# moabarar/nemar

Measured on AMD Instinct MI355X. Metric: train images/sec (256x256 A/B pairs), higher is better.
Workload: dtype f32

## Files before the change

### include/nemar_hip.h

```cpp
#ifndef NEMAR_HIP_H
#define NEMAR_HIP_H
#include <stddef.h>

#ifdef __cplusplus
extern "C" {
#endif

#define NEMAR_OK 0
#define NEMAR_EINVAL (-1)
#define NEMAR_ELAUNCH (-2)
#define NEMAR_EWORKSPACE (-3)

int nemar_version(void);
const char* nemar_last_error(void);

#define NEMAR_GRID_EXPLICIT 0
#define NEMAR_GRID_UNET 1
#define NEMAR_GRID_AFFINE 2
int nemar_grid_sample_fwd(const float* in, const float* grid_src, int grid_mode, float* out,
                          int N, int C, int H, int W, int Ho, int Wo, void* stream);
size_t nemar_grid_sample_bwd_workspace(int N, int C, int H, int W);
size_t nemar_grid_sample_bwd_zeroed_bytes(int N, int C, int H, int W);
int nemar_grid_sample_bwd(const float* in, const float* grid_src, int grid_mode, const float* gout,
                          float* gin, int accum_gin, float* ggrid, int accum_ggrid,
// ... 77 lines not shown
int nemar_conv2d_bwd_data_ex(const float* gy, const float* w, const float* bias, int act, float slope, float* gx0, int C0,
                             float* gx1, int C1, int N, int H, int W, int K, int OH, int OW, int R, int S, int stride, int pad,
                             int pad_mode, void* workspace, size_t ws_bytes, int prepacked, void* stream,
                             const nemar_conv_extras* extras);
int nemar_conv2d_bwd_weight_ex(const float* x0, int C0, const float* x1, int C1, const float* gy, float* gw, float* gb, int N,
                               int H, int W, int K, int OH, int OW, int R, int S, int stride, int pad, int pad_mode,
                               void* workspace, size_t ws_bytes, void* stream, const nemar_conv_extras* extras);
int nemar_pack_plan_record(int plan);
int nemar_pack_plan_jobs(int plan);
size_t nemar_pack_plan_bytes(int plan);
int nemar_pack_plan_dirty(int plan);
int nemar_pack_plan_commit(int plan, void* device_buffer, size_t bytes, void* stream);
int nemar_pack_plan_run(int plan, void* stream);
int nemar_pack_plan_reset(int plan);
int nemar_last_route(void);
int nemar_config_epoch(void);
int nemar_set_max_words_lazy(int on);
int nemar_max_words_finalize(void* max_words, int samples, void* stream);
size_t nemar_conv2d_scratch(int N, int H, int W, int K, int C, int R, int S, int stride, int pad);
int nemar_absmax(const float* t, long long n, void* out_word, void* stream);
int nemar_absmax_samples(const float* t, int samples, long long per_sample, void* out_words, void* stream);
int nemar_kernel_timer(int enable);
int nemar_kernel_timer_read(double* total_ms, double* total_flop, int* launches);
size_t nemar_bias_grad_workspace(int N, int C, int HW);
int nemar_bias_grad(const float* g, float* gb, int N, int C, int HW, void* workspace, size_t ws_bytes, void* stream);

int nemar_instnorm_fwd(const float* x, const float* residual, float* y, float* stats, int planes, int HW,
                       float eps, int act, float slope, void* stream);
int nemar_instnorm_bwd(const float* x, const float* stats, const float* gy, float* gx, int planes, int HW,
                       int act, float slope, void* stream);
// ... 108 lines not shown
```

### nemar_amd/_lib.py

```python
import ctypes as C
import os

import torch

_HERE = os.path.dirname(os.path.abspath(__file__))
PRODUCT_PATH = os.path.join(_HERE, "lib", "libnemar_hip.so")
AB_PATH = os.path.join(_HERE, "lib", "libnemar_hip_ab.so")
DEFAULT_PATH = AB_PATH if (os.environ.get("NEMAR_AB_LIBRARY") == "1" or os.environ.get("NEMAR_TUNE")) else PRODUCT_PATH

_f = C.POINTER(C.c_float)
_vp = C.c_void_p
_i = C.c_int
_fl = C.c_float
_sz = C.c_size_t
_ll = C.c_longlong
_db = C.c_double
_u64 = C.c_ulonglong
_u32 = C.c_uint

SIGNATURES = {
    "nemar_version": (_i, []),
    "nemar_last_error": (C.c_char_p, []),
    "nemar_grid_sample_fwd": (_i, [_vp, _vp, _i, _vp, _i, _i, _i, _i, _i, _i, _vp]),
    "nemar_grid_sample_bwd_workspace": (_sz, [_i, _i, _i, _i]),
# ... 20 lines not shown
    "nemar_conv2d_bwd_data_workspace": (_sz, [_i] * 10),
    "nemar_conv2d_bwd_data": (_i, [_vp, _vp, _vp, _i, _fl, _vp, _i, _vp, _i, _i, _i, _i, _i, _i, _i, _i, _i, _i, _i,
                                   _i, _vp, _sz, _i, _vp]),
    "nemar_conv2d_bwd_weight_workspace": (_sz, [_i] * 11),
    "nemar_conv2d_bwd_weight": (_i, [_vp, _i, _vp, _i, _vp, _vp, _vp, _i, _i, _i, _i, _i, _i, _i, _i, _i, _i, _i, _vp, _sz,
                                     _vp]),
    "nemar_conv2d_scratch": (_sz, [_i] * 9),
    "nemar_conv2d_gy_planes_bytes": (_sz, [_i] * 10),
    "nemar_absmax": (_i, [_vp, _ll, _vp, _vp]),
    "nemar_absmax_samples": (_i, [_vp, _i, _ll, _vp, _vp]),
    "nemar_kernel_timer": (_i, [_i]),
    "nemar_kernel_timer_read": (_i, [C.POINTER(C.c_double), C.POINTER(C.c_double), C.POINTER(_i)]),
    "nemar_bias_grad_workspace": (_sz, [_i, _i, _i]),
    "nemar_bias_grad": (_i, [_vp, _vp, _i, _i, _i, _vp, _sz, _vp]),
    "nemar_last_route": (_i, []),
    "nemar_last_gy_planes": (_i, []),
    "nemar_config_epoch": (_i, []),
    "nemar_set_max_words_lazy": (_i, [_i]),
    "nemar_instnorm_fwd": (_i, [_vp, _vp, _vp, _vp, _i, _i, _fl, _i, _fl, _vp]),
    "nemar_instnorm_bwd": (_i, [_vp, _vp, _vp, _vp, _i, _i, _i, _fl, _vp]),
    "nemar_instnorm_fwd_max": (_i, [_vp, _vp, _vp, _vp, _i, _i, _fl, _i, _fl, _vp, _i, _vp]),
    "nemar_instnorm_fwd_planes": (_i, [_vp, _vp, _vp, _vp, _vp, _i, _i, _i, _i, _fl, _i, _fl, _fl, _u64, _u32, _vp, _vp, _vp, _vp, _vp]),
    "nemar_instnorm_bwd_planes": (_i, [_vp, _vp, _vp, _vp, _i, _i, _i, _i, _i, _fl, _fl, _u64, _u32, _i, _vp, _vp, _vp, _vp, _vp, _vp]),
    "nemar_bias_from_partials": (_i, [_vp, _i, _i, _vp, _vp]),
    "nemar_conv2d_bwd_data_fusable": (_i, [_i] * 10),
    "nemar_conv2d_x_planes_bytes": (_sz, [_i] * 5),
    "nemar_set_dropout_base": (_i, [_vp]),
    "nemar_store_words": (_i, [_vp, _vp, _i, _vp]),
    "nemar_pack_plan_record": (_i, [_i]),
    "nemar_pack_plan_jobs": (_i, [_i]),
# ... 95 lines not shown
    def raw(self, name):
        return self._fns[name]

    def last_error(self):
        return self._fns["nemar_last_error"]().decode("utf-8", "replace")

    def __getattr__(self, name):
        fns = self.__dict__.get("_fns", {})
        full = name if name.startswith("nemar_") else "nemar_" + name
        if full not in fns:
            if full in AB_SIGNATURES:
                raise NemarHipError("%s has no %s: the measurement switches exist only in the -DNEMAR_AB build "
                                    "(libnemar_hip_ab.so; set NEMAR_AB_LIBRARY=1 before nemar_amd is imported)" % (self.__dict__.get("path"), full))
            raise AttributeError(name)
        fn = fns[full]
        if {**SIGNATURES, **AB_SIGNATURES}[full][0] is not _i or full in ("nemar_version", "nemar_last_route", "nemar_last_gy_planes", "nemar_config_epoch", "nemar_set_max_words_lazy", "nemar_pack_plan_jobs", "nemar_pack_plan_dirty", "nemar_conv2d_bwd_data_fusable", "nemar_conv2d_bwd_data_addend_ok"):
            return fn

        if os.environ.get("NEMAR_DEBUG_SYNC"):
            def checked(*a):
                import sys
                sys.stderr.write("[nemar] %s %s\n" % (full, [x for x in a if isinstance(x, (int, float))]))
                sys.stderr.flush()
                rc = fn(*a)
                torch.cuda.synchronize()
                if rc != 0:
                    raise NemarHipError("%s failed (%d): %s" % (full, rc, self.last_error()))
                return rc
            checked.__name__ = full
            self.__dict__[name] = checked
            return checked
# ... 27 lines not shown
```

### nemar_amd/csrc/conv.hip

```cpp
#define NEMAR_CONV_HIP
#include "common.h"
#include "conv_exact.h"
#include "conv_call.h"
#include "conv_route.h"
#include "pack_plan.h"

#ifdef NEMAR_AB
extern int g_split16_ring3;
extern int g_split16_ksplit_cap;
extern int g_narrow_fwd4;
extern int g_wg_xreg;
extern int g_register_vec4;
extern int g_overlap_per_lane;
extern int g_histogram_per_lane;
void nemar_norm_planes_debug(int bits);
#endif

int nemar_narrow_fwd(const float* x, const float* w, const float* bias, float* y, int N, int C, int H, int W, int K, int R,
                     int pad, int border, int act, float slope, float* part, size_t part_floats, hipStream_t st);
int nemar_narrow_wgrad(const float* x, const float* gy, float* gw, int N, int C, int H, int W, int K, int R, int pad,
                       int border, float* part, hipStream_t st);
void nemar_wgrad2_launch(const float* x0, int C0, const float* x1, int C1, const float* gy, float* gw, float* gb, int N,
                         int H, int W, int K, int OH, int OW, int R, int S, int stride, int pad, int pad_mode,
                         int target_blocks, bool vec_ok, int dbg, float* part, hipStream_t st);
void nemar_sum_partials_pair(const float* part_a, long long stride_a, int splits_a, float* dst_a, long long n_a,
                             const float* part_b, long long stride_b, int splits_b, float* dst_b, long long n_b, bool accumulate, hipStream_t st);
void nemar_sum_partials_fold(const float* part, long long stride, int splits, float* gx, long long planes, int H, int W, int pad,
                             const float* addend, hipStream_t st);
void nemar_sum_partials(const float* part, long long stride, int splits, float* dst, long long n, bool accumulate,
                        hipStream_t st);

namespace {

static thread_local int g_last_route = 0;
static thread_local int g_last_gy_planes = 0;
static NEMAR_SWITCH(int, g_config_epoch, 0);

struct WgradParams {
    const float* src0; const float* src1; int C0, C1, Hs, Ws;
    const float* gy; int K, OH, OW;
    float* gw; int J;
    float* gb;
    float* part;
    float* partb;
    int N, P, sy, sx, R, S, pad, border;
    int pix_per_split;
    int dbg;
    FastDiv fd_ohw, fd_ow;
};
// ... 458 lines not shown
    }
}

void k7_mf_run(const K7MfPlan& m_, const float* src, const float* w, int Ks, int Cb, int dgrad, const float* bias, float* out, int N, int H, int W,
               int fold, int act, float slope, float* wsf, int prepacked, hipStream_t st) {
    K7MfPlan m = m_;
    float* wt = wsf + m.wt_off;
    void* packed = wsf + m.pack_off;
    float* P = wsf + m.p_off;
    if (!prepacked) {
        K7MfWtArgs a{w, wt, Ks, Cb, dgrad, nemar_stream_grid(32 * Cb * 7, 256), 1};
        if (nemar_pack_recording()) nemar_pack_record_job(PACK_FAM_PRE, &a, a.gx, 1);
        hipLaunchKernelGGL(k7_mf_weights_kernel, dim3(a.gx), dim3(256), 0, st, w, wt, Ks, Cb, dgrad);
        nemar_s16g_pack(m.q, m.pl, wt, (long long)Cb * 7, 7, packed, st);
    }
    m.q.src0 = src; m.q.src1 = nullptr; m.q.dst0 = P; m.q.dst1 = nullptr; m.q.bias = nullptr; m.q.dbg = 0; m.q.tl = nullptr;
    nemar_s16g_conv(m.q, m.pl, packed, st);
    const long long total = (long long)N * Ks * H * W;
    hipLaunchKernelGGL(k7_mf_sum_kernel, dim3(nemar_stream_grid(total, 256)), dim3(256), 0, st, (const float*)P, bias, out, Ks, H, W, m.PH, m.PW, fold,
                       act, slope, total);
}

__global__ __launch_bounds__(256) void pad_planes_kernel(const float* __restrict__ src, float* __restrict__ dst, int plane,
                                                         int plane_padded, long long total) {
    for (long long idx = (long long)blockIdx.x * blockDim.x + threadIdx.x; idx < total;
         idx += (long long)gridDim.x * blockDim.x) {
        const long long pl = idx / plane_padded;
        const int r = (int)(idx - pl * plane_padded);
        dst[idx] = r < plane ? src[pl * plane + r] : 0.f;
    }
// ... 17 lines not shown
                      int act, float slope, void* workspace, size_t ws_bytes, int prepacked, void* stream) {
    NEMAR_CLEAR_HIP_ERROR();
    NEMAR_REQUIRE(x0 && w && y && workspace, "conv2d_fwd: null pointer");
    NEMAR_REQUIRE(C0 > 0 && C1 >= 0 && (C1 == 0 || x1), "conv2d_fwd: bad channel split %d+%d", C0, C1);
    NEMAR_REQUIRE(N > 0 && H > 0 && W > 0 && K > 0 && R > 0 && S > 0 && R * S <= MAX_TAPS, "conv2d_fwd: bad shape");
    NEMAR_REQUIRE(stride >= 1 && pad >= 0 && pad < 32768, "conv2d_fwd: bad stride/pad");
    NEMAR_REQUIRE(pad_mode == BORDER_ZERO || (pad_mode == BORDER_REFLECT && pad < H && pad < W),
                  "conv2d_fwd: reflect pad %d needs pad < H,W (%d,%d)", pad, H, W);
    const int C = C0 + C1;
    const int OH = (H + 2 * pad - R) / stride + 1, OW = (W + 2 * pad - S) / stride + 1;
    NEMAR_REQUIRE(OH > 0 && OW > 0, "conv2d_fwd: empty output");
    NEMAR_REQUIRE((long long)N * OH * OW < (1ll << 31) && (long long)C * H * W < (1ll << 31) && (long long)C * R * S < (1 << 20),
                  "conv2d_fwd: problem too large for 32-bit tile indexing");
    ConvFacts f = facts_of(call, bias, act, slope);
    FwdPlan P = plan_fwd({N, C0, C1, H, W, K, R, S, stride, pad, pad_mode}, f);
    if (ws_bytes < sizeof(float) * P.total) {
        nemar_set_error("conv2d_fwd: workspace %zu < %zu", ws_bytes, sizeof(float) * P.total);
        return NEMAR_EWORKSPACE;
    }
    hipStream_t st = (hipStream_t)stream;
    const char* what = "conv2d_fwd";
    g_last_route = P.route;
    switch (P.route) {
    case ROUTE_K7:
        if (P.sub == FwdPlan::K7_MANY_FEW) {
            k7_mf_run(P.k7, x0, w, K, C, 0, bias, y, N, H, W, 0, act, slope, (float*)workspace, prepacked, st);
            what = "conv2d_fwd (7x7 many -> few, 16-bit pipe)";
        } else {
            if (!prepacked) nemar_k7_fm_pack(w, (long long)C * 49, 49, 0, K, C, workspace, st);
            nemar_k7_fm_conv(x0, C, H, W, 3, pad_mode == BORDER_REFLECT, workspace, bias, y, K, N, H, W, act, slope, 0, st);
            what = "conv2d_fwd (7x7, 16-bit pipe)";
        }
        break;
    case ROUTE_NARROW:
        nemar_narrow_fwd(x0, w, bias, y, N, C, H, W, K, R, pad, pad_mode, act, slope,
                         g_deterministic ? (float*)workspace : nullptr, ws_bytes / sizeof(float), st);
        what = "conv2d_fwd (narrow)";
// ... 60 lines not shown
    NEMAR_REQUIRE(N > 0 && H > 0 && W > 0 && K > 0 && OH > 0 && OW > 0 && R * S <= MAX_TAPS && R > 0 && S > 0,
                  "conv2d_bwd_data: bad shape");
    NEMAR_REQUIRE(stride >= 1 && stride <= 4 && pad >= 0, "conv2d_bwd_data: bad stride/pad");
    NEMAR_REQUIRE((H + 2 * pad - R) / stride + 1 == OH && (W + 2 * pad - S) / stride + 1 == OW,
                  "conv2d_bwd_data: gy %dx%d inconsistent with x %dx%d k%d s%d p%d", OH, OW, H, W, R, stride, pad);
    const int C = C0 + C1;
    const bool refl = pad_mode == BORDER_REFLECT && pad > 0;
    NEMAR_REQUIRE(pad_mode != BORDER_REFLECT || (pad < H && pad < W), "conv2d_bwd_data: reflect pad too large");
    NEMAR_REQUIRE(!refl || (!bias && act == ACT_NONE && gx1 == nullptr),
                  "conv2d_bwd_data: reflect mode supports a single destination without bias/activation");
    NEMAR_REQUIRE(!refl || stride > 1 || pad <= 4, "conv2d_bwd_data: reflect pad %d > 4 unsupported", pad);
    ConvFacts f = facts_of(call, bias, act, slope);
    f.gx0 = gx0 != nullptr; f.gx1 = gx1 != nullptr;
    f.gy_planes_bytes = call.gy_planes_out ? call.gy_planes_bytes : 0;
    DgradPlan L = plan_dgrad({N, C0, C1, H, W, K, R, S, stride, pad, pad_mode}, f);
    if (ws_bytes < sizeof(float) * L.total) {
        nemar_set_error("conv2d_bwd_data: workspace %zu < %zu", ws_bytes, sizeof(float) * L.total);
        return NEMAR_EWORKSPACE;
    }
    NEMAR_REQUIRE((long long)N * (H + 2 * pad) * (W + 2 * pad) < (1ll << 31) && (long long)K * OH * OW < (1ll << 31) && (long long)K * R * S < (1 << 20),
                  "conv2d_bwd_data: problem too large for 32-bit tile indexing");
    hipStream_t st = (hipStream_t)stream;
    float* wsf = (float*)workspace;
    const long long total = (long long)N * C * H * W;
    const int mskip = L.mskip;
    const char* what = "conv2d_bwd_data";
    g_last_route = L.route;
    switch (L.sub) {
    case DgradPlan::K7_MANY_FEW:
        k7_mf_run(L.k7, gy, w, C, K, 1, nullptr, gx0, N, H, W, L.k7_fold, ACT_NONE, 0.f, wsf, prepacked, st);
        what = "conv2d_bwd_data (7x7 many -> few, 16-bit pipe)";
        break;
    case DgradPlan::K7_FEW_MANY:
        if (!prepacked) nemar_k7_fm_pack(w, 49, (long long)C * 49, 1, C, K, workspace, st);
        if (L.k7_fold == 2) {
            float* padded = wsf + ((nemar_k7_fm_pack_floats(C) + 3) & ~(size_t)3);
            nemar_k7_fm_conv(gy, K, OH, OW, 6, 0, workspace, nullptr, padded, C, N, H + 6, W + 6, ACT_NONE, 0.f, 0, st);
            fold_padded(padded, gx0, H, W, pad, total, nullptr, st);
        } else {
            nemar_k7_fm_conv(gy, K, OH, OW, L.k7_fold ? 6 : 3, 0, workspace, nullptr, gx0, C, N, H, W, ACT_NONE, 0.f, L.k7_fold, st);
        }
        what = "conv2d_bwd_data (7x7, 16-bit pipe)";
// ... 215 lines not shown
        p.pix_per_split = P.pix_per_split;
        p.part = part;
        p.partb = part ? part + P.bias_off : nullptr;
        const bool wide = K > 32;
        dim3 grid(nemar_cdiv(K, wide ? 128 : 32), nemar_cdiv(J, wide ? 128 : 256), P.splits), block(256);
        if (wide) hipLaunchKernelGGL((wgrad_kernel<2, 2, 2, 2>), grid, block, 0, st, p);
        else hipLaunchKernelGGL((wgrad_kernel<1, 4, 1, 2>), grid, block, 0, st, p);
        if (part) nemar_sum_partials_pair(part, (long long)K * J, P.splits, gw, (long long)K * J, gb ? p.partb : nullptr, K, P.splits, gb, K, true, st);
    }
    }
    NEMAR_CHECK_LAUNCH(what);
    return NEMAR_OK;
}

NEMAR_API int nemar_last_route(void) { return g_last_route; }
NEMAR_API int nemar_config_epoch(void) { return g_config_epoch; }

#ifdef NEMAR_AB
NEMAR_API int nemar_tune_ptr(void* p) { g_tl = (long long*)p; return NEMAR_OK; }

NEMAR_API int nemar_tune(int key, int value) {
    ++g_config_epoch;
    if (key == 0) { g_cfg128 = value; return NEMAR_OK; }
    if (key == 1) { g_lds_pad = value; return NEMAR_OK; }
    if (key == 2) { g_dbg = value; return NEMAR_OK; }
    if (key == 3) { g_narrow = value; return NEMAR_OK; }
    if (key == 4) { g_wgrad = value; return NEMAR_OK; }
    if (key == 6) { g_min_blocks = value > 0 ? value : 384; return NEMAR_OK; }
    if (key == 14) { g_deterministic = value != 0; return NEMAR_OK; }
    if (key == 8) { g_reflect_aux = value != 0; return NEMAR_OK; }
    if (key == 15) { g_xcd_map = value != 0; return NEMAR_OK; }
    if (key == 20) { g_split16 = value != 0; return NEMAR_OK; }
    if (key == 24) { g_s16g = value != 0; return NEMAR_OK; }
    if (key == 25) { g_s16g_min_mmac = value < 0 ? 0 : value; return NEMAR_OK; }
    if (key == 26) { g_s16g_wgrad_first = value != 0; return NEMAR_OK; }
    if (key == 27) { nemar_s16g_tune(0, value); return NEMAR_OK; }
    if (key == 29) { g_s16g_wgrad = value != 0; return NEMAR_OK; }
    if (key == 31) { nemar_norm_planes_debug(value); return NEMAR_OK; }
    if (key == 32) { g_split16_ring3 = value != 0; return NEMAR_OK; }
    if (key == 33) { g_k7 = value != 0; return NEMAR_OK; }
    if (key == 36) { g_split_act = value != 0; return NEMAR_OK; }
    if (key == 43) { g_fold_small = value != 0; return NEMAR_OK; }
    if (key == 37) { g_lds_claim = value; return NEMAR_OK; }
    if (key == 38) { g_wg_xreg = value != 0; return NEMAR_OK; }
    if (key == 39) { g_split16_ksplit_cap = value < 1 ? 1 : (value > 8 ? 8 : value); return NEMAR_OK; }
    if (key == 45) { g_overlap_per_lane = value != 0; return NEMAR_OK; }
    if (key == 46) { g_histogram_per_lane = value != 0; return NEMAR_OK; }
    if (key == 44) { g_register_vec4 = value != 0; return NEMAR_OK; }
    if (key == 47) { g_pointwise_rows = value != 0; return NEMAR_OK; }
    if (key == 35) { g_dual_gy = value != 0; return NEMAR_OK; }
    if (key == 34) { nemar_split16_wgrad_tune(value); return NEMAR_OK; }
    if (key == 30) { g_s16g_fold = value != 0; return NEMAR_OK; }
    if (key == 28) { nemar_s16g_tune(1, value); return NEMAR_OK; }
    if (key == 40) { nemar_s16g_tune(2, value); return NEMAR_OK; }
    if (key == 42) { nemar_s16g_tune(4, value); return NEMAR_OK; }
// ... 172 lines not shown
```

### nemar_amd/csrc/conv_k7.h

```cpp
#pragma once
#include <hip/hip_runtime.h>
#include <stddef.h>

bool nemar_k7_wgrad_eligible(int N, int C, int H, int W, int K, int R, int S, int stride, int pad);
int nemar_k7_wgrad_slabs(int N, int C, int H, int W, int K);
size_t nemar_k7_wgrad_floats(int N, int C, int H, int W, int K);
bool nemar_k7_wgrad(const float* x, const float* gy, float* gw, float* gb, int N, int C, int H, int W, int K, int pad_mode, float* part,
                    hipStream_t st);
void nemar_sum_partials(const float* part, long long stride, int splits, float* dst, long long n, bool accumulate, hipStream_t st);
void nemar_sum_partials_pair(const float* part_a, long long stride_a, int splits_a, float* dst_a, long long n_a,
                             const float* part_b, long long stride_b, int splits_b, float* dst_b, long long n_b, bool accumulate, hipStream_t st);


bool nemar_k7_fm_eligible(int Cs, int M, int R, int S, int stride, int pad);
size_t nemar_k7_fm_pack_floats(int M);
void nemar_k7_fm_pack(const float* w, long long wsm, long long wsc, int flip, int M, int Cs, void* packed, hipStream_t st);
void nemar_k7_fm_conv(const float* src, int Cs, int Hs, int Ws, int pad, int reflect, const void* packed, const float* bias, float* dst,
                      int M, int N, int Hv, int Wv, int act, float slope, int fold, hipStream_t st);
static inline bool nemar_k7_fm_fold_ok(int H, int W) { return H % 4 == 0 && H >= 8 && W % 64 == 0; }
```

### nemar_amd/csrc/conv_k7.hip

```cpp
#include "common.h"
#include "conv_k7.h"
#include "pack_plan.h"

namespace {

typedef float f32x16 __attribute__((ext_vector_type(16)));
typedef _Float16 f16x8 __attribute__((ext_vector_type(8)));
typedef _Float16 f16x2 __attribute__((ext_vector_type(2)));
typedef unsigned u32x4 __attribute__((ext_vector_type(4)));

constexpr int TEXP = 14;
constexpr int MODE_ZERO = 0, MODE_REFLECT = 1;

__device__ __forceinline__ float pow2f(int biased) {
    return biased < 1 ? 0.f : __builtin_bit_cast(float, (unsigned)(biased > 254 ? 254 : biased) << 23);
}
__device__ __forceinline__ int max_exponent(unsigned maxbits) {
    int e = (int)(maxbits >> 23);
    if (e < TEXP + 2) e = TEXP + 2;
    if (e > 254) e = 254;
    return e;
}
__device__ __forceinline__ void split8(const float* v, float s, u32x4& hi, u32x4& lo) {
#pragma unroll
// ... 585 lines not shown
K7WgGeom k7_wg_geom(int N, int C, int H, int W, int K) {
    K7WgGeom g;
    const bool stem = C <= 4;
    g.Hv = stem ? H : H + 6;
    g.Wv = stem ? W : W + 6;
    g.aligned = W % 32 == 0;
    g.strips = g.aligned ? W / 32 : nemar_cdiv(g.Wv, 8 * WG_KW);
    g.mblks = nemar_cdiv(stem ? K : C, 64);
    const long long cols = (long long)N * g.strips * g.mblks;
    int rblocks = (int)((512 + cols - 1) / cols);
    if (rblocks < 1) rblocks = 1;
    g.RB = (nemar_cdiv(g.Hv, rblocks) + 3) & ~3;
    if (g.RB < 8) g.RB = 8;
    g.rblocks = nemar_cdiv(g.Hv, g.RB);
    return g;
}

}

bool nemar_k7_wgrad_eligible(int N, int C, int H, int W, int K, int R, int S, int stride, int pad) {
    if (R != 7 || S != 7 || stride != 1 || pad != 3 || N <= 0 || H < 4 || W < 4) return false;
    const bool stem = C <= 4 && K % 32 == 0, head = K <= 4 && C % 32 == 0;
    return (stem || head) && (long long)N * (H + 12) * (W + 12) < (1ll << 30);
}

int nemar_k7_wgrad_slabs(int N, int C, int H, int W, int K) {
    const K7WgGeom g = k7_wg_geom(N, C, H, W, K);
    return N * g.rblocks * g.strips;
}

// ... 57 lines not shown
void nemar_k7_fm_conv(const float* src, int Cs, int Hs, int Ws, int pad, int reflect, const void* packed, const float* bias, float* dst,
                      int M, int N, int Hv, int Wv, int act, float slope, int fold, hipStream_t st) {
    K7FmParams p;
    p.small = K7View{src, Cs, Hs, Ws, pad, reflect ? MODE_REFLECT : MODE_ZERO};
    p.wp = (const u32x4*)packed;
    p.wmax = (const unsigned*)((const float*)packed + nemar_k7_fm_pack_floats(M) - 4);
    p.bias = bias; p.dst = dst; p.M = M; p.N = N; p.Hv = Hv; p.Wv = Wv; p.act = act; p.slope = slope;
    p.tiles_x = nemar_cdiv(Wv, FM_TW); p.tiles_y = nemar_cdiv(Hv, FM_RT); p.mblks = nemar_cdiv(M, 64);
    const long long ntiles = (long long)N * p.tiles_x * p.tiles_y;
    const int wgs = (int)(ntiles < 512 ? ntiles : 512) * p.mblks;
#define K7_FM(C_, F_) hipLaunchKernelGGL((k7_fm_kernel<C_, F_>), dim3(wgs), dim3(256), 0, st, p)
    if (fold) { if (Cs == 1) K7_FM(1, true); else if (Cs == 2) K7_FM(2, true); else if (Cs == 3) K7_FM(3, true); else K7_FM(4, true); }
    else { if (Cs == 1) K7_FM(1, false); else if (Cs == 2) K7_FM(2, false); else if (Cs == 3) K7_FM(3, false); else K7_FM(4, false); }
#undef K7_FM
}
```

### nemar_amd/csrc/conv_route.h

```cpp
#pragma once
#ifndef NEMAR_CONV_HIP
#error "conv_route.h holds conv.hip's own switches: include it from conv.hip only"
#endif
#include "common.h"
#include "conv_exact.h"
#include "conv_split16.h"
#include "conv_s16g.h"
#include "conv_k7.h"

bool nemar_narrow_eligible(int K, int C1, int R, int S, int stride, int N, int OH, int OW);
int nemar_narrow_wgrad_splits(int N, int C, int OH, int OW);
bool nemar_wgrad2_eligible(int K, int OH, int OW, bool gy_aligned16);
void nemar_wgrad2_plan(int K, int J, int P, int target_blocks, int* splits_out, int* pix_per_split_out);

using namespace nemar_exact;

namespace {

static NEMAR_SWITCH(int, g_split16, 1);
static NEMAR_SWITCH(long long, g_split16_min_mmac, 2000);
static NEMAR_SWITCH(int, g_split16_variant, 4);
static NEMAR_SWITCH(int, g_k7, 1);
static NEMAR_SWITCH(int, g_s16g, 1);
static NEMAR_SWITCH(long long, g_s16g_min_mmac, 30);
static NEMAR_SWITCH(int, g_s16g_wgrad, 1);
static NEMAR_SWITCH(int, g_s16g_wgrad_first, 0);
static NEMAR_SWITCH(int, g_s16g_fold, 1);
static NEMAR_SWITCH(int, g_split_act, 1);
static NEMAR_SWITCH(int, g_fold_small, 1);
static NEMAR_SWITCH(int, g_dual_gy, 1);
static NEMAR_SWITCH(int, g_reflect_aux, 1);
static NEMAR_SWITCH(int, g_deterministic, 1);
static NEMAR_SWITCH(int, g_ksplit, 1);
static NEMAR_SWITCH(int, g_narrow, 1);
static NEMAR_SWITCH(int, g_wgrad, 0);
static NEMAR_SWITCH(int, g_wgrad_blocks, 512);

// ... 113 lines not shown
    for (int ph = 0; ph < stride; ++ph)
        for (int pw = 0; pw < stride; ++pw) {
            TapTable t;
            dgrad_taps(t, R, S, pad, stride, ph, pw);
            const int OHc = (H - ph + stride - 1) / stride, OWc = (W - pw + stride - 1) / stride;
            if (t.n == 0 || OHc <= 0 || OWc <= 0 || t.n > (stride > 1 ? S16G_CLS_TAPS : S16G_MAX_TAPS)) return false;
            s16g_set_class(q, q.ncls++, t, OHc, OWc, ph, pw);
        }
    pl = nemar_s16g_plan(q);
    return pl.ok != 0;
}

struct K7MfPlan {
    S16gProblem q;
    S16gPlan pl;
    size_t wt_off, pack_off, p_off, total;
    int PH, PW;
    bool ok;
};
K7MfPlan k7_mf_plan(int N, int Cb, int Hs, int Ws, int spad, int border) {
    K7MfPlan m;
    m.ok = false;
    m.PH = Hs + 2 * spad - 6;
    m.PW = Ws + 2 * spad;
    S16gProblem& q = m.q;
    q = S16gProblem();
    q.C0 = Cb; q.C1 = 0; q.Hs = Hs; q.Ws = Ws; q.N = N; q.M = 32; q.M0 = 32;
    q.act = ACT_NONE; q.slope = 0.f; q.border = border; q.sstride = 1;
    q.OHf = m.PH; q.OWf = m.PW; q.osy = 1; q.osx = 1; q.ncls = 1;
    TapTable t;
    t.n = 7;
    for (int i = 0; i < 7; ++i) { t.dy[i] = (short)(i - spad); t.dx[i] = (short)(-spad); t.dyx[i] = ((i - spad) << 16) | ((-spad) & 0xffff); t.wofs[i] = i; }
    s16g_set_class(q, 0, t, m.PH, m.PW, 0, 0);
    m.pl = nemar_s16g_plan(q);
    if (!m.pl.ok) return m;
    m.wt_off = 0;
    m.pack_off = ((size_t)32 * Cb * 7 + 3) & ~(size_t)3;
    m.p_off = (m.pack_off + (nemar_s16g_pack_bytes(q, m.pl) + 3) / 4 + 3) & ~(size_t)3;
    m.total = m.p_off + (size_t)N * 32 * m.PH * m.PW;
    m.ok = true;
    return m;
}
bool k7_mf_eligible(int Cb, int Ks, int R, int S, int stride, int pad) {
    return g_k7 && R == 7 && S == 7 && stride == 1 && pad == 3 && Ks >= 1 && Ks <= 4 && Cb >= 16 && Cb % 16 == 0;
}

struct FwdPlan {
    int route;
    enum Sub { PLAIN, K7_MANY_FEW, K7_FEW_MANY, SPLIT, SPLIT_ACT } sub;
    size_t pack, slab_off, total;
    int ksplit;
    K7MfPlan k7;
    S16gProblem q; S16gPlan pl;
};
// ... 1 lines not shown
    FwdPlan P;
    const int N = s.N, H = s.H, W = s.W, K = s.K, C = s.C(), R = s.R, S = s.S, stride = s.stride, pad = s.pad, OH = s.OH(), OW = s.OW();
    P.pack = packed_floats(K, C * R * S);
    if (wide_candidates(s).fwd)
        grow(P.pack, (nemar_split16_pack_bytes(K, C, R) + 3) / 4);
    if (s16g_fwd_problem(P.q, P.pl, N, C, 0, H, W, K, R, S, stride, pad, BORDER_ZERO, ACT_NONE, 0.f))
        grow(P.pack, (nemar_s16g_pack_bytes(P.q, P.pl) + 3) / 4);
    const bool k7_fm = nemar_k7_fm_eligible(C, K, R, S, stride, pad);
    if (k7_fm) grow(P.pack, nemar_k7_fm_pack_floats(K));
    P.ksplit = 1;
    if (g_ksplit && OH > 0 && OW > 0 && K > 4) P.ksplit = normalize_ksplit(C * R * S, small_problem_split(K, N * OH * OW, C * R * S));
    P.slab_off = (P.pack + 3) & ~(size_t)3;
    P.total = P.slab_off + (P.ksplit > 1 ? (size_t)P.ksplit * N * K * OH * OW : 0);
    P.k7.ok = false;
    if (k7_mf_eligible(C, K, R, S, stride, pad)) {
        P.k7 = k7_mf_plan(N, C, H, W, 3, BORDER_ZERO);
        if (P.k7.ok) grow(P.total, P.k7.total);
        if (s.pad_mode != BORDER_ZERO) P.k7 = k7_mf_plan(N, C, H, W, 3, s.pad_mode);
    }
    const int mode = s.pad_mode == BORDER_REFLECT ? SPLIT16_REFLECT : SPLIT16_ZERO;
    P.sub = FwdPlan::PLAIN;
    if (s.C1 == 0 && P.k7.ok) { P.route = ROUTE_K7; P.sub = FwdPlan::K7_MANY_FEW; }
    else if (g_k7 && s.C1 == 0 && f.act != ACT_TANH && k7_fm) { P.route = ROUTE_K7; P.sub = FwdPlan::K7_FEW_MANY; }
    else if (nemar_narrow_eligible(K, s.C1, R, S, stride, N, OH, OW) && g_narrow) P.route = ROUTE_NARROW;
    else if (g_split16 && s.C1 == 0 && f.act == ACT_NONE && split16_worth_it(N, OH, OW, K, C, R, S) &&
             nemar_split16_eligible(N, H, W, K, C, R, S, stride, pad, mode, g_split16_variant) &&
             f.scratch_bytes && f.scratch_bytes >= nemar_split16_scratch_total(N, H, W, K, C, OH, OW)) P.route = ROUTE_SPLIT16;
    else if (s16g_fwd_problem(P.q, P.pl, N, s.C0, s.C1, H, W, K, R, S, stride, pad, s.pad_mode, f.act, f.slope)) P.route = ROUTE_S16G;
    else {
        const bool split_act = g_split_act && (f.act == ACT_RELU || f.act == ACT_LRELU);
        P.route = ROUTE_EXACT;
        if (P.ksplit > 1 && (f.act == ACT_NONE || split_act)) P.sub = split_act ? FwdPlan::SPLIT_ACT : FwdPlan::SPLIT;
    }
// ... 68 lines not shown
            }
        }
        if (L.ksplit == 1) L.ksplit = small_problem_split(C, P, Kred);
        L.ksplit = normalize_ksplit(Kred, L.ksplit);
    }
    L.slab_off = o;
    if (L.ksplit > 1) o += (size_t)L.ksplit * N * C * Hs * Wsl;
    const bool aux = L.ring && pad == 1 && R == 3 && S == 3;
    L.aux_rows_off = o;
    if (aux) o += 6ull * N * K * W;
    L.aux_cols_off = o;
    if (aux) o += 8ull * N * K * H;
    L.total = o;
    L.k7.ok = false;
    if (k7_mf_eligible(K, C, R, S, stride, pad)) {
        L.k7 = k7_mf_plan(N, K, OH, OW, refl ? 6 : 3, BORDER_ZERO);
        if (L.k7.ok) grow(L.total, L.k7.total);
    }
    const bool k7_fm = C > 4 && nemar_k7_fm_eligible(K, C, R, S, stride, pad);
    if (k7_fm) grow(L.total, ((nemar_k7_fm_pack_floats(C) + 3) & ~(size_t)3) + (refl ? (size_t)N * C * (H + 6) * (W + 6) : 0));
    const bool one_plain = s.C1 == 0 && f.gx0 && !f.bias && f.act == ACT_NONE;
    const int mode = refl ? SPLIT16_DGRAD_REFLECT : SPLIT16_ZERO;
    L.mskip = f.gx0 ? 0 : s.C0;
    const bool own_problem = L.mskip != 0 || f.act == ACT_TANH;
    L.k7_fold = 0; L.want_gy_planes = false; L.gy_planes_need = 0; L.split16_ksplit = 0; L.narrow = L.split = L.aux_rows = false;
    if (one_plain && L.k7.ok) {
        L.route = ROUTE_K7; L.sub = DgradPlan::K7_MANY_FEW; L.k7_fold = refl ? 1 : 0;
    } else if (g_k7 && one_plain && k7_fm) {
        L.route = ROUTE_K7; L.sub = DgradPlan::K7_FEW_MANY; L.k7_fold = !refl ? 0 : nemar_k7_fm_fold_ok(H, W) ? 1 : 2;
    } else if (g_split16 && one_plain && split16_worth_it(N, OH, OW, K, C, R, S) &&
               nemar_split16_eligible(N, H, W, C, K, R, S, stride, pad, mode, g_split16_variant) &&
// ... 107 lines not shown
```

Measured before the change: 293.2.

## Fuse k7 many-to-few conv into a single MFMA kernel with in-LDS tap reduction

Adds a fused kernel for 7x7 convolutions with many input and few output channels. It loads input tiles with halos, splits them into fp16 hi/lo pairs with a dynamic exponent scale, and runs MFMA over the seven row taps. The column-tap diagonal sum, reflect folding, bias and activation are done from LDS before a single store. This removes the separate s16g conv pass, its large intermediate P buffer with the matching global write and read, and the follow-up reduction launch, and it shrinks the required workspace. In exchange the kernel is complex, with exponent rescaling and border-mirror logic that could hurt accuracy or correctness.

```diff
diff --git a/include/nemar_hip.h b/include/nemar_hip.h
--- a/include/nemar_hip.h
+++ b/include/nemar_hip.h
@@ -115,6 +115,7 @@
 int nemar_pack_plan_run(int plan, void* stream);
 int nemar_pack_plan_reset(int plan);
 int nemar_last_route(void);
+int nemar_last_k7_form(void);
 int nemar_config_epoch(void);
 int nemar_set_max_words_lazy(int on);
 int nemar_max_words_finalize(void* max_words, int samples, void* stream);
diff --git a/nemar_amd/_lib.py b/nemar_amd/_lib.py
--- a/nemar_amd/_lib.py
+++ b/nemar_amd/_lib.py
@@ -58,6 +58,7 @@
     "nemar_bias_grad_workspace": (_sz, [_i, _i, _i]),
     "nemar_bias_grad": (_i, [_vp, _vp, _i, _i, _i, _vp, _sz, _vp]),
     "nemar_last_route": (_i, []),
+    "nemar_last_k7_form": (_i, []),
     "nemar_last_gy_planes": (_i, []),
     "nemar_config_epoch": (_i, []),
     "nemar_set_max_words_lazy": (_i, [_i]),
@@ -183,7 +184,7 @@
                                     "(libnemar_hip_ab.so; set NEMAR_AB_LIBRARY=1 before nemar_amd is imported)" % (self.__dict__.get("path"), full))
             raise AttributeError(name)
         fn = fns[full]
-        if {**SIGNATURES, **AB_SIGNATURES}[full][0] is not _i or full in ("nemar_version", "nemar_last_route", "nemar_last_gy_planes", "nemar_config_epoch", "nemar_set_max_words_lazy", "nemar_pack_plan_jobs", "nemar_pack_plan_dirty", "nemar_conv2d_bwd_data_fusable", "nemar_conv2d_bwd_data_addend_ok"):
+        if {**SIGNATURES, **AB_SIGNATURES}[full][0] is not _i or full in ("nemar_version", "nemar_last_route", "nemar_last_k7_form", "nemar_last_gy_planes", "nemar_config_epoch", "nemar_set_max_words_lazy", "nemar_pack_plan_jobs", "nemar_pack_plan_dirty", "nemar_conv2d_bwd_data_fusable", "nemar_conv2d_bwd_data_addend_ok"):
             return fn
 
         if os.environ.get("NEMAR_DEBUG_SYNC"):
diff --git a/nemar_amd/csrc/conv.hip b/nemar_amd/csrc/conv.hip
--- a/nemar_amd/csrc/conv.hip
+++ b/nemar_amd/csrc/conv.hip
@@ -33,6 +33,7 @@
 namespace {
 
 static thread_local int g_last_route = 0;
+static thread_local int g_last_k7_form = 0;
 static thread_local int g_last_gy_planes = 0;
 static NEMAR_SWITCH(int, g_config_epoch, 0);
 
@@ -521,6 +522,12 @@
         hipLaunchKernelGGL(k7_mf_weights_kernel, dim3(a.gx), dim3(256), 0, st, w, wt, Ks, Cb, dgrad);
         nemar_s16g_pack(m.q, m.pl, wt, (long long)Cb * 7, 7, packed, st);
     }
+    if (m.fused) {
+        g_last_k7_form = 2;
+        nemar_k7_mf_fused(src, Cb, fold ? 6 : 3, m.q.border == BORDER_REFLECT, fold, packed, bias, out, Ks, N, H, W, act, slope, st);
+        return;
+    }
+    g_last_k7_form = 1;
     m.q.src0 = src; m.q.src1 = nullptr; m.q.dst0 = P; m.q.dst1 = nullptr; m.q.bias = nullptr; m.q.dbg = 0; m.q.tl = nullptr;
     nemar_s16g_conv(m.q, m.pl, packed, st);
     const long long total = (long long)N * Ks * H * W;
@@ -568,13 +575,15 @@
                   "conv2d_fwd: problem too large for 32-bit tile indexing");
     ConvFacts f = facts_of(call, bias, act, slope);
     FwdPlan P = plan_fwd({N, C0, C1, H, W, K, R, S, stride, pad, pad_mode}, f);
-    if (ws_bytes < sizeof(float) * P.total) {
-        nemar_set_error("conv2d_fwd: workspace %zu < %zu", ws_bytes, sizeof(float) * P.total);
+    const size_t ws_need = (P.route == ROUTE_K7 && P.sub == FwdPlan::K7_MANY_FEW && P.k7.fused) ? P.k7.need : P.total;
+    if (ws_bytes < sizeof(float) * ws_need) {
+        nemar_set_error("conv2d_fwd: workspace %zu < %zu", ws_bytes, sizeof(float) * ws_need);
         return NEMAR_EWORKSPACE;
     }
     hipStream_t st = (hipStream_t)stream;
     const char* what = "conv2d_fwd";
     g_last_route = P.route;
+    g_last_k7_form = 0;
     switch (P.route) {
     case ROUTE_K7:
         if (P.sub == FwdPlan::K7_MANY_FEW) {
@@ -665,8 +674,9 @@
     f.gx0 = gx0 != nullptr; f.gx1 = gx1 != nullptr;
     f.gy_planes_bytes = call.gy_planes_out ? call.gy_planes_bytes : 0;
     DgradPlan L = plan_dgrad({N, C0, C1, H, W, K, R, S, stride, pad, pad_mode}, f);
-    if (ws_bytes < sizeof(float) * L.total) {
-        nemar_set_error("conv2d_bwd_data: workspace %zu < %zu", ws_bytes, sizeof(float) * L.total);
+    const size_t ws_need = (L.route == ROUTE_K7 && L.sub == DgradPlan::K7_MANY_FEW && L.k7.fused) ? L.k7.need : L.total;
+    if (ws_bytes < sizeof(float) * ws_need) {
+        nemar_set_error("conv2d_bwd_data: workspace %zu < %zu", ws_bytes, sizeof(float) * ws_need);
         return NEMAR_EWORKSPACE;
     }
     NEMAR_REQUIRE((long long)N * (H + 2 * pad) * (W + 2 * pad) < (1ll << 31) && (long long)K * OH * OW < (1ll << 31) && (long long)K * R * S < (1 << 20),
@@ -677,6 +687,7 @@
     const int mskip = L.mskip;
     const char* what = "conv2d_bwd_data";
     g_last_route = L.route;
+    g_last_k7_form = 0;
     switch (L.sub) {
     case DgradPlan::K7_MANY_FEW:
         k7_mf_run(L.k7, gy, w, C, K, 1, nullptr, gx0, N, H, W, L.k7_fold, ACT_NONE, 0.f, wsf, prepacked, st);
@@ -922,6 +933,7 @@
 }
 
 NEMAR_API int nemar_last_route(void) { return g_last_route; }
+NEMAR_API int nemar_last_k7_form(void) { return g_last_k7_form; }
 NEMAR_API int nemar_config_epoch(void) { return g_config_epoch; }
 
 #ifdef NEMAR_AB
@@ -947,6 +959,7 @@
     if (key == 31) { nemar_norm_planes_debug(value); return NEMAR_OK; }
     if (key == 32) { g_split16_ring3 = value != 0; return NEMAR_OK; }
     if (key == 33) { g_k7 = value != 0; return NEMAR_OK; }
+    if (key == 48) { g_k7_fused = value != 0; return NEMAR_OK; }
     if (key == 36) { g_split_act = value != 0; return NEMAR_OK; }
     if (key == 43) { g_fold_small = value != 0; return NEMAR_OK; }
     if (key == 37) { g_lds_claim = value; return NEMAR_OK; }
diff --git a/nemar_amd/csrc/conv_k7.h b/nemar_amd/csrc/conv_k7.h
--- a/nemar_amd/csrc/conv_k7.h
+++ b/nemar_amd/csrc/conv_k7.h
@@ -18,3 +18,10 @@
 void nemar_k7_fm_conv(const float* src, int Cs, int Hs, int Ws, int pad, int reflect, const void* packed, const float* bias, float* dst,
                       int M, int N, int Hv, int Wv, int act, float slope, int fold, hipStream_t st);
 static inline bool nemar_k7_fm_fold_ok(int H, int W) { return H % 4 == 0 && H >= 8 && W % 64 == 0; }
+
+
+bool nemar_k7_mf_fused_eligible(int N, int Cb, int H, int W, int fold);
+void nemar_k7_mf_fused(const float* src, int Cb, int spad, int reflect, int fold, const void* packed, const float* bias, float* dst, int Ks,
+                       int N, int H, int W, int act, float slope, hipStream_t st);
+int nemar_k7_mf_tile_w();
+int nemar_k7_mf_tile_rows();
diff --git a/nemar_amd/csrc/conv_k7.hip b/nemar_amd/csrc/conv_k7.hip
--- a/nemar_amd/csrc/conv_k7.hip
+++ b/nemar_amd/csrc/conv_k7.hip
@@ -623,6 +623,289 @@
     if (g.RB < 8) g.RB = 8;
     g.rblocks = nemar_cdiv(g.Hv, g.RB);
     return g;
+}
+
+constexpr int MF_TW = 64, MF_RT = 7;
+constexpr int MF_PW = MF_TW + 6, MF_HR = MF_RT + 6, MF_GPR = (MF_TW + 8) / 4, MF_HCP = 4 * MF_GPR, MF_HP16 = MF_HR * MF_HCP;
+constexpr int MF_NT = 4, MF_NP = 128 * MF_NT;
+constexpr int MF_AW16 = 7 * 4 * 32;
+constexpr int MF_PSTR = MF_NP + 8;
+constexpr int MF_LDS16 = MF_AW16 + 4 * MF_HP16;
+static_assert(MF_RT * MF_PW <= MF_NP && 32 * MF_PSTR * 4 <= MF_LDS16 * 16, "the P tile fits the accumulators and the operand regions");
+static_assert(MF_HR * MF_GPR <= 256 && 2 * MF_LDS16 * 16 <= 160 * 1024 - 1024, "two loader slots per thread; two workgroups per CU");
+typedef float f32x4u __attribute__((ext_vector_type(4), aligned(4)));
+
+struct K7MfParams {
+    const float* src;
+    const u32x4* wp;
+    const unsigned* wmax;
+    const float* bias;
+    float* dst;
+    int Cb, Hs, Ws, N, Ks, H, W;
+    int spad, reflect, fold, act;
+    float slope;
+    int tiles_x, tiles_y, nchunks, vec, xcd;
+};
+
+__device__ __forceinline__ int mf_mirror_clamp(int i, int n) {
+    i = i < 0 ? -i : i;
+    i = i >= n ? 2 * (n - 1) - i : i;
+    return i < 0 ? 0 : (i >= n ? n - 1 : i);
+}
+
+__global__ __launch_bounds__(256, 2) void k7_mf_fused_kernel(K7MfParams p) {
+#ifdef NEMAR_HOST_EMULATION
+    __shared__ __attribute__((aligned(16))) u32x4 smem[MF_LDS16];
+#else
+    extern __shared__ __attribute__((aligned(16))) u32x4 smem[];
+#endif
+    __shared__ unsigned red[4];
+    u32x4* const As = smem;
+    u32x4* const Bs = smem + MF_AW16;
+    float* const Pt = reinterpret_cast<float*>(smem);
+    const int tid = threadIdx.x, wid = __builtin_amdgcn_readfirstlane(tid >> 6), lane = tid & 63, l31 = lane & 31, lhi = lane >> 5;
+    int t = blockIdx.x;
+    if (p.xcd) t = (t & 7) * ((int)gridDim.x >> 3) + (t >> 3);
+    const int txi = t % p.tiles_x;
+    t /= p.tiles_x;
+    const int tyi = t % p.tiles_y, n = t / p.tiles_y;
+    const int x0 = txi * MF_TW;
+    int Y0 = tyi * MF_RT, nr, ya, yb;
+    if (p.fold) {
+        if (tyi == p.tiles_y - 1) { Y0 = p.H - 1; nr = MF_RT; ya = p.H - 4; yb = p.H; }
+        else { nr = min(MF_RT, p.H - 1 - Y0); ya = max(0, Y0 - 3); yb = min(Y0 + nr - 3, p.H - 4); }
+    } else {
+        nr = min(MF_RT, p.H - Y0); ya = Y0; yb = Y0 + nr;
+    }
+    const size_t HWs = (size_t)p.Hs * p.Ws;
+
+    const int kgl = wid >> 1;
+    int soff[2], lpos[2], mirr[2];
+    bool smirr[2], sdead[2];
+#pragma unroll
+    for (int i = 0; i < 2; ++i) {
+        const int gp = (tid & 127) + 128 * i;
+        soff[i] = 0; lpos[i] = -1; mirr[i] = 0;
+        if (gp < MF_HR * MF_GPR) {
+            const int hr = gp / MF_GPR, g = gp - hr * MF_GPR;
+            int iy = Y0 + hr - p.spad;
+            const int ixg = x0 - 4 + 4 * g;
+            bool ok = ixg >= 0 && ixg < p.Ws && hr < nr + 6;
+            if (p.reflect) iy = mf_mirror_clamp(iy, p.Hs);
+            else ok = ok && (unsigned)iy < (unsigned)p.Hs;
+            if (ok) {
+                soff[i] = iy * p.Ws + ixg;
+                lpos[i] = kgl * MF_HP16 + hr * MF_HCP + 4 * g;
+                if (p.reflect) {
+                    const int nl = ixg == 0 ? 3 : 0;
+                    const int nrt = ixg == p.Ws - 4 ? min(3, 4 * (MF_GPR - 1 - g)) : 0;
+                    mirr[i] = nl | (nrt << 2);
+                }
+            }
+        }
+        smirr[i] = __any(mirr[i] != 0) != 0;
+        sdead[i] = __any(lpos[i] < 0) != 0;
+    }
+    for (int w = tid; w < 4 * MF_HP16; w += 256) Bs[w] = u32x4{0u, 0u, 0u, 0u};
+    f32x4u v[2][8];
+    u32x4 wq[4];
+#define K7MF_LOAD(ch_)                                                                                                  \
+    {                                                                                                                   \
+        const float* const cb_ = p.src + ((size_t)n * p.Cb + (ch_) * 16 + kgl * 8) * HWs;                               \
+        _Pragma("unroll") for (int i = 0; i < 2; ++i)                                                                   \
+            _Pragma("unroll") for (int j = 0; j < 8; ++j) v[i][j] = *reinterpret_cast<const f32x4u*>(cb_ + (size_t)j * HWs + soff[i]); \
+         \
+        _Pragma("unroll") for (int i = 0; i < 4; ++i) wq[i] = p.wp[(size_t)(ch_) * MF_AW16 + min(tid + 256 * i, MF_AW16 - 1)]; \
+    }
+
+    int bbase[MF_NT];
+#pragma unroll
+    for (int nt = 0; nt < MF_NT; ++nt) {
+        const int px = wid * (32 * MF_NT) + 32 * nt + l31;
+        int py = px / MF_PW, pj = px - py * MF_PW;
+        if (py >= MF_RT) { py = 0; pj = 0; }
+        bbase[nt] = lhi * MF_HP16 + py * MF_HCP + pj + 1;
+    }
+    const int abase = lhi * 32 + l31;
+    f32x16 acc[MF_NT];
+#pragma unroll
+    for (int nt = 0; nt < MF_NT; ++nt)
+#pragma unroll
+        for (int r = 0; r < 16; ++r) acc[nt][r] = 0.f;
+
+    int E = 0;
+    K7MF_LOAD(0)
+    for (int chunk = 0; chunk < p.nchunks; ++chunk) {
+#pragma unroll
+        for (int i = 0; i < 2; ++i)
+            if (sdead[i]) {
+#pragma unroll
+                for (int j = 0; j < 8; ++j)
+                    if (lpos[i] < 0) v[i][j] = f32x4u{0.f, 0.f, 0.f, 0.f};
+            }
+        {
+            float mf = 0.f;
+#pragma unroll
+            for (int i = 0; i < 2; ++i)
+#pragma unroll
+                for (int j = 0; j < 8; ++j)
+                    mf = fmaxf(fmaxf(mf, fmaxf(__builtin_fabsf(v[i][j][0]), __builtin_fabsf(v[i][j][1]))),
+                               fmaxf(__builtin_fabsf(v[i][j][2]), __builtin_fabsf(v[i][j][3])));
+            unsigned m = __builtin_bit_cast(unsigned, mf);
+            if (m >= 0x7f800000u) {
+                m = 0;
+#pragma unroll
+                for (int i = 0; i < 2; ++i)
+#pragma unroll
+                    for (int j = 0; j < 8; ++j)
+#pragma unroll
+                        for (int e = 0; e < 4; ++e) {
+                            const unsigned u = __builtin_bit_cast(unsigned, (float)v[i][j][e]) & 0x7fffffffu;
+                            m = max(m, u < 0x7f800000u ? u : 0u);
+                        }
+            }
+            m = wave_max_to_lane63(m);
+            if (lane == 63) red[wid] = m;
+        }
+        __builtin_amdgcn_s_waitcnt(0xC07F);
+        __builtin_amdgcn_s_barrier();
+#pragma unroll
+        for (int i = 0; i < 4; ++i)
+            if (tid + 256 * i < MF_AW16) As[tid + 256 * i] = wq[i];
+        {
+            const int e = max_exponent(max(max(red[0], red[1]), max(red[2], red[3])));
+            if (e > E) {
+                if (chunk > 0) {
+                    const float f = pow2f(127 + E - e);
+#pragma unroll
+                    for (int nt = 0; nt < MF_NT; ++nt)
+#pragma unroll
+                        for (int r = 0; r < 16; ++r) acc[nt][r] *= f;
+                }
+                E = e;
+            }
+        }
+        {
+            const float scale = pow2f(127 + TEXP + 127 - E);
+#pragma unroll
+            for (int i = 0; i < 2; ++i) {
+                if (lpos[i] < 0) continue;
+#pragma unroll
+                for (int e = 0; e < 4; ++e) {
+                    float t8[8];
+#pragma unroll
+                    for (int j = 0; j < 8; ++j) t8[j] = v[i][j][e];
+                    u32x4 hi, lo;
+                    split8(t8, scale, hi, lo);
+                    Bs[lpos[i] + e] = hi;
+                    Bs[2 * MF_HP16 + lpos[i] + e] = lo;
+                    if (smirr[i]) {
+                        const int nl = mirr[i] & 3, nrt = mirr[i] >> 2;
+                        if (e >= 1 && e <= nl) {
+                            Bs[lpos[i] - e] = hi;
+                            Bs[2 * MF_HP16 + lpos[i] - e] = lo;
+                        }
+                        if (e <= 2 && 3 - e <= nrt) {
+                            Bs[lpos[i] + 6 - e] = hi;
+                            Bs[2 * MF_HP16 + lpos[i] + 6 - e] = lo;
+                        }
+                    }
+                }
+            }
+        }
+        if (chunk + 1 < p.nchunks) K7MF_LOAD(chunk + 1)
+        __builtin_amdgcn_s_waitcnt(0xC07F);
+        __builtin_amdgcn_s_barrier();
+#pragma unroll
+        for (int tap = 0; tap < 7; ++tap) {
+            const u32x4 ah = As[(tap * 2 + 0) * 64 + abase], al = As[(tap * 2 + 1) * 64 + abase];
+            u32x4 bh[MF_NT], bl[MF_NT];
+#pragma unroll
+            for (int nt = 0; nt < MF_NT; ++nt) {
+                bh[nt] = Bs[bbase[nt] + tap * MF_HCP];
+                bl[nt] = Bs[2 * MF_HP16 + bbase[nt] + tap * MF_HCP];
+            }
+#pragma unroll
+            for (int nt = 0; nt < MF_NT; ++nt)
+                acc[nt] = __builtin_amdgcn_mfma_f32_32x32x16_f16(__builtin_bit_cast(f16x8, al), __builtin_bit_cast(f16x8, bh[nt]), acc[nt], 0, 0, 0);
+#pragma unroll
+            for (int nt = 0; nt < MF_NT; ++nt)
+                acc[nt] = __builtin_amdgcn_mfma_f32_32x32x16_f16(__builtin_bit_cast(f16x8, ah), __builtin_bit_cast(f16x8, bl[nt]), acc[nt], 0, 0, 0);
+#pragma unroll
+            for (int nt = 0; nt < MF_NT; ++nt)
+                acc[nt] = __builtin_amdgcn_mfma_f32_32x32x16_f16(__builtin_bit_cast(f16x8, ah), __builtin_bit_cast(f16x8, bh[nt]), acc[nt], 0, 0, 0);
+        }
+    }
+#undef K7MF_LOAD
+
+    unsigned wm = 0;
+    {
+        const u32x4* const q = reinterpret_cast<const u32x4*>(p.wmax);
+#pragma unroll
+        for (int i = 0; i < NEMAR_PACK_MAX_PARTS / 4; ++i) {
+            const u32x4 w4 = q[i];
+            wm = max(max(wm, w4[0]), max(max(w4[1], w4[2]), w4[3]));
+        }
+    }
+    const float u1 = pow2f(E - TEXP), u2 = 1.f / pow2f(127 + TEXP + 127 - max_exponent(wm));
+    const float u12 = u1 * u2;
+    const bool one_mul = u12 != 0.f && u12 < 3.0e38f;
+    __builtin_amdgcn_s_waitcnt(0xC07F);
+    __builtin_amdgcn_s_barrier();
+#pragma unroll
+    for (int nt = 0; nt < MF_NT; ++nt) {
+        const int px = wid * (32 * MF_NT) + 32 * nt + l31;
+#pragma unroll
+        for (int r = 0; r < 16; ++r) {
+            const int m = (r & 3) + 8 * (r >> 2) + 4 * lhi;
+            Pt[m * MF_PSTR + px] = one_mul ? acc[nt][r] * u12 : (acc[nt][r] * u1) * u2;
+        }
+    }
+    __builtin_amdgcn_s_waitcnt(0xC07F);
+    __builtin_amdgcn_s_barrier();
+
+    const int nrows = yb - ya, rowoff = p.fold ? 3 : 0;
+    const size_t dplane = (size_t)p.H * p.W;
+    for (int it = tid; it < p.Ks * nrows * (MF_TW / 4); it += 256) {
+        const int cg = it & (MF_TW / 4 - 1), rest = it / (MF_TW / 4), yl = rest % nrows, k = rest / nrows;
+        const int y = ya + yl, xg = x0 + 4 * cg;
+        if (xg >= p.W) continue;
+        const float* const Pk = Pt + (k * 8) * MF_PSTR;
+        auto at = [&](int ry, int jb, int lo, int hi) {
+            const float* const r = Pk + ry * MF_PW + jb;
+            float s = 0.f;
+#pragma unroll
+            for (int dx = 0; dx < 7; ++dx)
+                if (dx >= lo && dx <= hi) s += r[dx * MF_PSTR + dx];
+            return s;
+        };
+        float o[4];
+#pragma unroll
+        for (int e = 0; e < 4; ++e) {
+            const int x = xg + e, jc = x - x0;
+            float vv;
+            if (!p.fold) {
+                vv = at(y - Y0, jc, 0, 6);
+            } else {
+                const int y1 = (y >= 1 && y <= 3) ? 3 - y : -1, y2 = (y <= p.H - 2 && y >= p.H - 4) ? 2 * (p.H - 1) - y + 3 : -1;
+                const bool m1 = x >= 1 && x <= 3, m2 = x <= p.W - 2 && x >= p.W - 4;
+                auto row = [&](int ry) {
+                    float s = at(ry, jc, 0, 6);
+                    if (m1) s += at(ry, -x, x + 3, 6);
+                    if (m2) s += at(ry, 2 * p.W - 2 - x - x0, 0, x - p.W + 4);
+                    return s;
+                };
+                vv = row(y + rowoff - Y0);
+                if (y1 >= 0) vv += row(y1 - Y0);
+                if (y2 >= 0) vv += row(y2 - Y0);
+            }
+            if (p.bias) vv += p.bias[k];
+            o[e] = p.act == 1 ? fmaxf(vv, 0.f) : (p.act == 2 ? (vv > 0.f ? vv : vv * p.slope) : (p.act == 3 ? tanhf(vv) : vv));
+        }
+        float* const d = p.dst + ((size_t)n * p.Ks + k) * dplane + (size_t)y * p.W + xg;
+        if (p.vec) *reinterpret_cast<float4*>(d) = make_float4(o[0], o[1], o[2], o[3]);
+        else { d[0] = o[0]; d[1] = o[1]; d[2] = o[2]; d[3] = o[3]; }
+    }
 }
 
 }
@@ -710,3 +993,35 @@
     else { if (Cs == 1) K7_FM(1, false); else if (Cs == 2) K7_FM(2, false); else if (Cs == 3) K7_FM(3, false); else K7_FM(4, false); }
 #undef K7_FM
 }
+
+int nemar_k7_mf_tile_w() { return MF_TW; }
+int nemar_k7_mf_tile_rows() { return MF_RT; }
+
+bool nemar_k7_mf_fused_eligible(int N, int Cb, int H, int W, int fold) {
+    if (N <= 0 || Cb < 16 || Cb % 16 != 0 || H < 1 || W < 8 || W % 4 != 0) return false;
+    if (fold && H < 2 * MF_RT - 6) return false;
+    const long long tiles = (long long)N * nemar_cdiv(W, MF_TW) * (fold ? nemar_cdiv(H - 1, MF_RT) + 1 : nemar_cdiv(H, MF_RT));
+    return tiles < (1ll << 30) && (long long)(H + 12) * (W + 12) < (1ll << 30);
+}
+
+void nemar_k7_mf_fused(const float* src, int Cb, int spad, int reflect, int fold, const void* packed, const float* bias, float* dst, int Ks,
+                       int N, int H, int W, int act, float slope, hipStream_t st) {
+    K7MfParams p;
+    p.src = src; p.Cb = Cb; p.Hs = H; p.Ws = W; p.N = N; p.Ks = Ks; p.H = H; p.W = W;
+    p.nchunks = Cb / 16;
+    p.wp = (const u32x4*)packed;
+    p.wmax = (const unsigned*)(p.wp + (size_t)p.nchunks * MF_AW16);
+    p.bias = bias; p.dst = dst;
+    p.spad = spad; p.reflect = reflect; p.fold = fold; p.act = act; p.slope = slope;
+    p.tiles_x = nemar_cdiv(W, MF_TW);
+    p.tiles_y = fold ? nemar_cdiv(H - 1, MF_RT) + 1 : nemar_cdiv(H, MF_RT);
+    p.vec = (reinterpret_cast<uintptr_t>(dst) & 15) == 0 ? 1 : 0;
+    const dim3 grid(p.tiles_x * p.tiles_y * N), block(256);
+    p.xcd = grid.x % 8 == 0 ? 1 : 0;
+#ifdef NEMAR_HOST_EMULATION
+    hipLaunchKernelGGL(k7_mf_fused_kernel, grid, block, 0, st, p);
+#else
+    const size_t lds = nemar_lds_bytes(reinterpret_cast<const void*>(&k7_mf_fused_kernel), (size_t)MF_LDS16 * 16, false);
+    hipLaunchKernelGGL(k7_mf_fused_kernel, grid, block, lds, st, p);
+#endif
+}
diff --git a/nemar_amd/csrc/conv_route.h b/nemar_amd/csrc/conv_route.h
--- a/nemar_amd/csrc/conv_route.h
+++ b/nemar_amd/csrc/conv_route.h
@@ -21,6 +21,7 @@
 static NEMAR_SWITCH(long long, g_split16_min_mmac, 2000);
 static NEMAR_SWITCH(int, g_split16_variant, 4);
 static NEMAR_SWITCH(int, g_k7, 1);
+static NEMAR_SWITCH(int, g_k7_fused, 1);
 static NEMAR_SWITCH(int, g_s16g, 1);
 static NEMAR_SWITCH(long long, g_s16g_min_mmac, 30);
 static NEMAR_SWITCH(int, g_s16g_wgrad, 1);
@@ -164,13 +165,15 @@
 struct K7MfPlan {
     S16gProblem q;
     S16gPlan pl;
-    size_t wt_off, pack_off, p_off, total;
+    size_t wt_off, pack_off, p_off, total, need;
     int PH, PW;
     bool ok;
-};
-K7MfPlan k7_mf_plan(int N, int Cb, int Hs, int Ws, int spad, int border) {
+    bool fused;
+};
+K7MfPlan k7_mf_plan(int N, int Cb, int Hs, int Ws, int spad, int border, bool fold) {
     K7MfPlan m;
     m.ok = false;
+    m.fused = false;
     m.PH = Hs + 2 * spad - 6;
     m.PW = Ws + 2 * spad;
     S16gProblem& q = m.q;
@@ -187,7 +190,9 @@
     m.wt_off = 0;
     m.pack_off = ((size_t)32 * Cb * 7 + 3) & ~(size_t)3;
     m.p_off = (m.pack_off + (nemar_s16g_pack_bytes(q, m.pl) + 3) / 4 + 3) & ~(size_t)3;
+    m.fused = g_k7_fused && nemar_k7_mf_fused_eligible(N, Cb, Hs, Ws, fold ? 1 : 0);
     m.total = m.p_off + (size_t)N * 32 * m.PH * m.PW;
+    m.need = m.fused ? m.p_off : m.total;
     m.ok = true;
     return m;
 }
@@ -219,9 +224,9 @@
     P.total = P.slab_off + (P.ksplit > 1 ? (size_t)P.ksplit * N * K * OH * OW : 0);
     P.k7.ok = false;
     if (k7_mf_eligible(C, K, R, S, stride, pad)) {
-        P.k7 = k7_mf_plan(N, C, H, W, 3, BORDER_ZERO);
+        P.k7 = k7_mf_plan(N, C, H, W, 3, BORDER_ZERO, false);
         if (P.k7.ok) grow(P.total, P.k7.total);
-        if (s.pad_mode != BORDER_ZERO) P.k7 = k7_mf_plan(N, C, H, W, 3, s.pad_mode);
+        if (s.pad_mode != BORDER_ZERO) P.k7 = k7_mf_plan(N, C, H, W, 3, s.pad_mode, false);
     }
     const int mode = s.pad_mode == BORDER_REFLECT ? SPLIT16_REFLECT : SPLIT16_ZERO;
     P.sub = FwdPlan::PLAIN;
@@ -320,7 +325,7 @@
     L.total = o;
     L.k7.ok = false;
     if (k7_mf_eligible(K, C, R, S, stride, pad)) {
-        L.k7 = k7_mf_plan(N, K, OH, OW, refl ? 6 : 3, BORDER_ZERO);
+        L.k7 = k7_mf_plan(N, K, OH, OW, refl ? 6 : 3, BORDER_ZERO, refl);
         if (L.k7.ok) grow(L.total, L.k7.total);
     }
     const bool k7_fm = C > 4 && nemar_k7_fm_eligible(K, C, R, S, stride, pad);
```

Measured after the change: 294.8, median of 6. No clear change (+0.6%).
